# stulacy/bmm-mcmc

Measured on AMD Instinct MI355X. Metric: gibbs_sweeps_per_s, higher is better.
Workload: dtype f64; 1 GPU; c5: gibbs_collapsed K=20 N=10000000 P=100, 1 chain per GPU; sampler=collapsed, K=20, N=10000000, P=100, batch=2500000, chains=1, chains_per_gpu=1, burn_sweeps=30, x_layout=bit planes, ceil(P/32) words per observation, packed once at hand-over

## Files before the change

bmm-mcmc_amd/csrc/bmm_spec.h:

```cpp
#pragma once
#include <stdint.h>

#include "bmm_exp256.h"

#if defined(__HIPCC__)
#include <hip/hip_runtime.h>
#define BMM_HD __host__ __device__ __forceinline__
#else
#define BMM_HD inline
#endif

namespace bmm {

constexpr int kGroupW = 5;
constexpr int kGroupWAlt = 4;
constexpr int kGroupWm = 3;
constexpr int kGroupMm = 1 << kGroupWm;
constexpr int kOwnSub = 6;

enum : uint32_t {
    kStreamZ = 0,
    kStreamStickA = 1,
    kStreamStickB = 2,
    kStreamThetaA = 3,
// ... 326 lines not shown
    return n;
}

constexpr float kPkEpsUnit = 3.2f * 0x1p-24f;
constexpr float kPkLnCats = 4.1588831f;
BMM_HD float pk_band(float m, int G, float unit) {
    return unit * (80.0f + (float)(G + 2) * (__builtin_fabsf(m) + kPkLnCats + 1.0f));
}
template <int KT, class Exp2 = Exp2Fast>
BMM_HD bool draw_pk(const float (&sc)[KT], float m, double u, int G, float unit, int& cnt, Exp2 ex2 = Exp2()) {
    static_assert(KT <= kTier1MaxCats, "the band is derived for at most kTier1MaxCats categories");
    float c[KT];
    float run = 0.0f;
#if defined(__HIP_DEVICE_COMPILE__)
#pragma unroll
#endif
    for (int k = 0; k < KT; ++k) {
        run = run + ex2((sc[k] - m) * 0x1.715476p+0f);
        c[k] = run;
    }
    const float t = (float)u * run;
    float nearest = __builtin_inff();
    int n = 0;
#if defined(__HIP_DEVICE_COMPILE__)
#pragma unroll
#endif
    for (int k = 0; k < KT; ++k) {
        const float diff = t - c[k];
        n += diff >= 0.0f ? 1 : 0;
        nearest = __builtin_fminf(nearest, __builtin_fabsf(diff));
    }
    cnt = n;
    return nearest > pk_band(m, G, unit) * run && m > -__builtin_inff() && m < __builtin_inff();
}

BMM_HD double rnorm_(Stream& st) {
    for (;;) {
        const U4 r = st.next();
        const double v1 = 2.0 * u01(r.x, r.y) - 1.0, v2 = 2.0 * u01(r.z, r.w) - 1.0;
        const double s = v1 * v1 + v2 * v2;
        if (s < 1.0 && s > 0.0) return v1 * sqrt_(div_(-2.0 * log_(s), s));
    }
}

BMM_HD double rgamma_(double shape, Stream& st) {
    if (!(shape > 0.0)) return 0.0;
    double boost = 1.0;
    if (shape < 1.0) {
        const U4 r = st.next();
        boost = exp_(div_(log_(u01_open0(r.x, r.y)), shape));
        shape = shape + 1.0;
    }
    const double d = shape - 0.33333333333333331483;
    const double c = div_(1.0, sqrt_(9.0 * d));
    for (;;) {
        const double x = rnorm_(st);
        double v = 1.0 + c * x;
        if (v <= 0.0) continue;
        v = v * v * v;
        const U4 r = st.next();
        const double u = u01_open0(r.x, r.y);
        const double x2 = x * x;
        if (log_(u) < 0.5 * x2 + d - d * v + d * log_(v)) return d * v * boost;
    }
}

// ... 296 lines not shown
```

bmm-mcmc_amd/csrc/chain.hip:

```cpp
#include <hip/hip_runtime.h>
#include <hip/hip_ext.h>
#include <rccl/rccl.h>

#include <dlfcn.h>
#include <emmintrin.h>
#include <sched.h>
#include <sys/mman.h>

#include <algorithm>
#include <cmath>
#include <cstdarg>
#include <cstdio>
#include <cstdint>
#include <cstdlib>
#include <cstring>
#include <atomic>
#include <chrono>
#include <condition_variable>
#include <exception>
#include <functional>
#include <limits>
#include <memory>
#include <mutex>
#include <new>
// ... 428 lines not shown
    resample_fn fn = nullptr, fn_emit = nullptr;
    int grid_max_emit = 0;

    const int32_t* dX = nullptr;
    int32_t* dX_owned = nullptr;
    uint32_t* dXb = nullptr;
    struct Planes { uint32_t* d = nullptr; size_t bytes = 0; std::atomic<int> refs{1}; };
    Planes* planes = nullptr;
    bool xb_borrowed = false;
    bool bits = false;
    int num_cus = 0;
    char *arena = nullptr, *run_arena = nullptr;
    size_t arena_bytes = 0, run_arena_bytes = 0;
    int32_t* dZ[2] = {nullptr, nullptr};
    int32_t *dNk = nullptr, *dS = nullptr, *dDNk = nullptr, *dDS = nullptr;
    double *dAlpha = nullptr, *dTab = nullptr, *dPi = nullptr, *dTheta = nullptr;
    bool have_data = false, have_init = false, started = false;
    int sweep = 0;

    int burnin = 0, S = 0;
    int32_t* dTrace = nullptr;
    double *dThetaTrace = nullptr, *dAlphaTrace = nullptr, *dPiTrace = nullptr;
    char* dOutBlk[2] = {nullptr, nullptr};
    size_t out_blk_bytes = 0;

    int32_t* dNkTrace = nullptr;
    int nk_trace_base = 0;
    unsigned long long* dDiag = nullptr;
    int* dViable = nullptr;
    int* dSelfDone = nullptr;
    int32_t *dDNkAlt = nullptr, *dDSAlt = nullptr;
    unsigned long long* dPkStat = nullptr;
    int pk_defer_every = 0;
    int* dDbgFlag = nullptr;
    int64_t predM = 0;
    uint32_t* dXnb = nullptr;
    double *dPredTab = nullptr, *dPredMax = nullptr, *dPredSum = nullptr, *dRespAcc = nullptr;
    bool pred_resp = false;
    int pred_folded = 0;
    score_fn pfn = nullptr;
    int pred_grid_max = 0;
    size_t pred_lds = 0;
    SweepTrace pred_rec;
    int64_t pred_cells = 0;
    uint32_t* dPnMb = nullptr;
    int64_t *dPnRow = nullptr, *dPnOff = nullptr;
    int32_t* dPnCol = nullptr;
    double *dCellMax = nullptr, *dCellSum = nullptr, *dSplitTab = nullptr, *dPnScratch = nullptr;
    int64_t pn_scratch_stride = 0;
    na_score_fn pn_fn = nullptr;
    int pn_grid_max = 0;
    size_t pn_lds = 0;
    bool loo_on = false;
    double *dLooTab = nullptr, *dLooAcc = nullptr, *dLooOut = nullptr;
    bool loo_generic = false;
    double* dLooScratch = nullptr;
    int64_t loo_scratch_stride = 0;
    int loo_folded = 0;
    score_fn lfn = nullptr;
    int loo_minus = 0, loo_grid_max = 0;
    size_t loo_lds = 0;
    SweepTrace loo_rec;
    int sm_moves = 0, sm_scans = 0, sm_sets = 0;
    uint8_t *dSmSide = nullptr, *dSmSideLaunch = nullptr;
    double* dSmLq = nullptr;
    int32_t* dSmStat = nullptr;
// ... 203 lines not shown
    int flag = 0;
    hipError_t e = hipGetLastError();
    if (e == hipSuccess) e = hipMemcpyAsync(&flag, dflag, sizeof(int), hipMemcpyDeviceToHost, c->stream);
    if (e == hipSuccess) e = hipStreamSynchronize(c->stream);
    if (e != hipSuccess) return set_err(BMM_E_HIP, "validating X failed: %s", hipGetErrorString(e));
    if (flag) return set_err(BMM_E_ARG, "data must be binary: X holds a value other than 0 and 1");
    return BMM_OK;
}

constexpr int64_t kLargeN = (int64_t)1 << 16;
int64_t default_batch(int sampler, int64_t N) {
    if (sampler == BMM_SAMPLER_SB || sampler == BMM_SAMPLER_FULL) return N;
    const int64_t div = N >= kLargeN ? 4 : (sampler == BMM_SAMPLER_DP ? 16 : 8);
    const int64_t b = N / div;
    return b < 1 ? 1 : b;
}

TableLayout layout_of(const bmm_chain* c) { return layout_of(c->p, !explicit_params(c->p.mode)); }

int dbg_env_int(const char* name, int unset) { const char* v = dbg_env(name); return v ? (atoi(v) > 0 ? atoi(v) : 0) : unset; }
struct DebugSwitches {
    bool generic = dbg_env("BMM_DEBUG_GENERIC");
    bool int32_layout = dbg_env("BMM_X_LAYOUT_INT32");
    int cus = dbg_env_int("BMM_DEBUG_CUS", 0);
    int threads = dbg_env_int("BMM_DEBUG_THREADS", -1);
    bool split = dbg_env("BMM_DEBUG_SPLIT");
    bool nosplit = dbg_env("BMM_DEBUG_NOSPLIT");
    bool small = dbg_env("BMM_DEBUG_SMALL");
    bool noself = dbg_env("BMM_DEBUG_NOSELF");
    bool nopk = dbg_env("BMM_DEBUG_NOPK");
    bool pk = dbg_env("BMM_DEBUG_PK");
    bool nopipe = dbg_env("BMM_DEBUG_PK_NOPIPE");
    int pk_defer_every = dbg_env_int("BMM_DEBUG_PK_DEFER_EVERY", 0);
};

struct ChainShape {
    ChainParams p{};
    int64_t batch = 1;
    bool generic = false;
    int minus_in_lds = 1;
    size_t lds_bytes_base = 0;
};
ChainParams geometry(int sampler, int P, int K, int kt, int W) {
    ChainParams q{};
    q.mode = sampler; q.P = P; q.K = K; q.KT = kt; q.W = W;
    q.G = (P + W - 1) / W; q.Gm = (P + kGroupWm - 1) / kGroupWm;
    q.Kc = sampler == BMM_SAMPLER_DP ? K + 1 : K;
    return q;
}
size_t image_bytes(const ChainParams& q, bool own_tables) {
    const TableLayout l = layout_of(q, own_tables && !explicit_params(q.mode));
    return (size_t)(own_tables ? l.doubles() : l.head()) * sizeof(double) + ((size_t)q.K * q.P + q.K + 4) * sizeof(int32_t);
}

size_t pk_image_bytes(const ChainParams& q) {
    const TableLayout l = layout_of(q, true);
    return (size_t)(2 * pk_tq_doubles(l) + l.tm() - l.nk()) * sizeof(double) + ((size_t)q.K * q.P + q.K + 4 + kPkQueue) * sizeof(int32_t);
}

int group_width_rule(int sampler, int K, int P) {
    const int kt = pick_kt(sampler == BMM_SAMPLER_DP ? K + 1 : K);
    if (kt < 0 || P > kMaxP) return kGroupWAlt;
    return image_bytes(geometry(sampler, P, K, kt, kGroupW), true) <= kLdsMax ? kGroupW : kGroupWAlt;
}

int64_t generic_threads(int Kc) {
// ... 120 lines not shown
    int rc = chain_stream_create(c, true);
    if (rc) { c->stream = old; c->stream_kind = old_kind; return rc; }
    chain_stream_release(c->device, old, old_kind);
    return BMM_OK;
}

struct Carver {
    char* base;
    size_t used = 0;
    template <class T> T* take(size_t n) {
        const size_t off = (used + 255) & ~(size_t)255;
        used = off + n * sizeof(T);
        return base ? reinterpret_cast<T*>(base + off) : nullptr;
    }
};

int chain_alloc(bmm_chain* c) {
    const ChainParams& p = c->p;
    HIP_TRY(hipSetDevice(c->device));
    {
        int rcs = chain_stream_create(c, false);
        if (rcs) return rcs;
    }
    const size_t nz = (size_t)p.N;
    const size_t ns = (size_t)p.K * p.P, nn = (size_t)p.K;
    const size_t ntab = (size_t)layout_of(c).doubles() + (explicit_params(p.mode) ? 0 : 2 * (size_t)pk_tq_doubles(layout_of(c)));
    auto carve = [&](Carver& a) {
        c->dNk = a.take<int32_t>(nn);
        c->dDNk = a.take<int32_t>(nn * kDeltaReps);
        c->dS = a.take<int32_t>(ns);
        c->dDS = a.take<int32_t>(ns * kDeltaReps);
        c->dTab = a.take<double>(ntab);
#ifdef BMM_DIAG
        c->dDiag = a.take<unsigned long long>(18);
#endif
        c->dSelfDone = a.take<int>(1);
        c->dViable = a.take<int>(1);
        c->dDNkAlt = a.take<int32_t>(nn * kDeltaReps);
        c->dDSAlt = a.take<int32_t>(ns * kDeltaReps);
#ifdef BMM_DEBUG_HOOKS
        c->dDbgFlag = a.take<int>(1);
        c->dPkStat = a.take<unsigned long long>(3);
#endif
        const size_t zeroed = a.used;
        c->dAlpha = a.take<double>(1);
        c->dPi = a.take<double>(nn);
        c->dTheta = a.take<double>(ns);
        c->dZ[0] = a.take<int32_t>(nz);
        c->dZ[1] = a.take<int32_t>(nz);
        return zeroed;
    };
    Carver measure{nullptr};
    carve(measure);
    c->arena = static_cast<char*>(dev_pool().get(c->device, measure.used, &c->arena_bytes));
    if (!c->arena) return set_err(BMM_E_HIP, "allocating the chain's state failed: %s", hipGetErrorString(hipGetLastError()));
    Carver real{c->arena};
    const size_t zeroed = carve(real);
    if (c->generic) HIP_TRY(hipMalloc(&c->dScratch, (size_t)c->scratch_stride * p.Kc * sizeof(double)));
    HIP_TRY(hipMemsetAsync(c->arena, 0, zeroed, c->stream));
    HIP_TRY(hipMemsetAsync(c->dZ[0], 0xff, nz * sizeof(int32_t), c->stream));
    HIP_TRY(hipMemcpyAsync(c->dAlpha, &c->alpha0, sizeof(double), hipMemcpyHostToDevice, c->stream));
    HIP_TRY(hipStreamSynchronize(c->stream));
    return BMM_OK;
}

int dbg_labels_ok(bmm_chain* c) {
#ifdef BMM_DEBUG_HOOKS
    int flag = 0;
    HIP_TRY(hipMemcpy(&flag, c->dDbgFlag, sizeof(int), hipMemcpyDeviceToHost));
    if (flag) return set_err(BMM_E_STATE, "a resample kernel produced or read a label outside [0, K): kernel bug (debug-hooks build check)");
#else
    (void)c;
#endif
    return BMM_OK;
}

int launch_resample(bmm_chain* c, const int32_t* z_in, int32_t* z_out, int64_t lo, int64_t hi,
                    uint32_t sweep) {
    ResampleArgs a{};
    a.X = c->dX; a.Xb = c->dXb; a.z_in = z_in; a.z_out = z_out; a.tab = c->dTab; a.dNk = c->dDNk; a.dS = c->dDS;
    a.lo = lo; a.hi = hi; a.sweep = sweep; a.minus_in_lds = c->minus_in_lds; a.diag = c->dDiag;
    a.dbg_flag = c->dDbgFlag; a.dbg_inject = (dbg_env("BMM_DEBUG_BADLABEL") ? 1 : 0) | (dbg_env("BMM_DEBUG_STRAGGLER") ? 2 : 0) |
                                             (dbg_env("BMM_DEBUG_DRAW_FALLBACK") ? 4 : 0) | (dbg_env("BMM_DEBUG_DRAW_NOEPS") ? 8 : 0) |
                                             (dbg_env("BMM_DEBUG_PK_GENKEY") ? 16 : 0);
    a.Nk = c->dNk; a.S = c->dS; a.alpha_ptr = c->dAlpha; a.self_done = c->dSelfDone;
#ifdef BMM_DEBUG_HOOKS
    a.pk_stat = c->dPkStat;
    a.pk_defer_every = c->pk_defer_every;
#endif
    const bool emit = c->probs_dst != nullptr;
    const bool use_generic = c->generic || (emit && !c->fn_emit);
    const bool self_launch = c->form.self && !emit && !use_generic;
    if (self_launch) { a.dNk_prev = c->dDNk; a.dS_prev = c->dDS; a.dNk = c->dDNkAlt; a.dS = c->dDSAlt; }
    const KernelForm& form = emit ? c->form_emit : c->form;
    const int gmax = emit ? c->grid_max_emit : c->grid_max;
    const int64_t ntiles = use_generic ? 1 : (hi - lo + tile_of(form) - 1) / tile_of(form);
    int grid = (int)(ntiles < gmax ? ntiles : gmax);
    if (use_generic) {
        const int64_t nt256 = (hi - lo + 255) / 256;
        const int64_t maxb = c->scratch_stride / 256;
        grid = (int)(nt256 < maxb ? nt256 : maxb);
    }
    if (emit) { a.wts = c->dWts; a.wtot = c->dWtot; }
    if (form.pk && !use_generic) {
        a.Xb += lo;
        if (a.z_in) a.z_in += lo;
        a.z_out += lo;
    }
    hipEvent_t e0 = nullptr, e1 = nullptr;
    if (c->prof > 0 && sweep % (uint32_t)c->prof == 0) {
        if (c->ev_used + 2 > c->ev.size()) {
            hipEvent_t a0, a1;
            HIP_TRY(hipEventCreate(&a0));
            HIP_TRY(hipEventCreate(&a1));
            c->ev.push_back(a0); c->ev.push_back(a1);
        }
        e0 = c->ev[c->ev_used]; e1 = c->ev[c->ev_used + 1];
        c->ev_used += 2;
    }
    if (use_generic) {
        if (e0) hipExtLaunchKernelGGL(k_resample_generic, dim3(grid), dim3(256), 0, c->stream, e0, e1, 0, c->p, a,
// ... 923 lines not shown
        return set_err(BMM_E_ARG, "Error: sampler currently not implemented for non-symmetric priors on beta and gamma");
    if (sampler == BMM_SAMPLER_DP && K < 2) return set_err(BMM_E_ARG, "maxK must be >= 2");
    if (alpha < 0.0) return set_err(BMM_E_ARG, "alpha must be >= 0 (0 = sample it)");
    int ndev = 0;
    if (hipGetDeviceCount(&ndev) != hipSuccess || ndev < 1)
        return set_err(BMM_E_NODEVICE, "no HIP device visible; this path has no CPU fallback");
    const int slot = device;
    if (const int fake = fake_devices()) {
        if (device < 0 || device >= fake) return set_err(BMM_E_ARG, "device %d out of range (have %d)", device, fake);
        device = device % ndev;
    }
    if (device < 0 || device >= ndev) return set_err(BMM_E_ARG, "device %d out of range (have %d)", device, ndev);

    bmm_chain* c = new (std::nothrow) bmm_chain();
    if (!c) return set_err(BMM_E_ARG, "out of host memory");
    const DebugSwitches dbg;
    const ChainShape shape = chain_shape(sampler, N, P, K, batch, dbg);
    ChainParams& p = c->p;
    p = shape.p;
    p.beta = beta; p.gamma = gamma; p.a = a; p.b = b; p.seed = seed;
    p.sample_alpha = alpha == 0.0;
    c->alpha0 = p.sample_alpha ? 1.0 : alpha;
    c->device = device;
    c->slot = slot;
    c->batch = shape.batch;
    if (p.Kc > kMaxCatsAny) {
        delete c;
        return set_err(BMM_E_UNSUPPORTED, "%d categories exceed the %d this build supports", p.Kc, kMaxCatsAny);
    }
    const int cus = device_cus(device);
    if (cus <= 0) { delete c; return set_err(BMM_E_HIP, "hipGetDeviceProperties failed"); }
    c->bits = !dbg.int32_layout;
    c->pk_defer_every = dbg.pk_defer_every;
    c->generic = shape.generic;
    c->minus_in_lds = shape.minus_in_lds;
    c->lds_bytes_base = c->lds_bytes = shape.lds_bytes_base;
    if (c->generic) {
        c->form = KernelForm{p.KT, 256, tier_of(c), c->bits, 1, false, p.W, false};
        c->scratch_stride = generic_threads(p.Kc);
        c->grid_max = (int)(c->scratch_stride / 256);
    } else {
        c->num_cus = dbg.cus >= 1 ? dbg.cus : cus;
        rc = pick_kernel(c);
        if (rc) { delete c; return rc; }
    }
    rc = chain_alloc(c);
    if (rc) { bmm_chain_destroy(c); return rc; }
    *out = c;
    return BMM_OK;
}

void bmm_chain_destroy(bmm_chain* c) {
    if (!c) return;
    (void)hipSetDevice(c->device);
    if (c->stream) (void)hipStreamSynchronize(c->stream);
#ifdef BMM_DIAG
    if (c->dDiag) {
        unsigned long long d[18] = {};
        const bool ok = hipMemcpy(d, c->dDiag, sizeof d, hipMemcpyDeviceToHost) == hipSuccess;
        if (ok && d[5] && d[0]) {
            const double tot = (double)(d[0] + d[1] + d[2] + d[3] + d[4]);
            fprintf(stderr, "[bmm diag] waves=%llu cycles/wave: score %.0f (%.1f%%) pack %.0f (%.1f%%) draw %.0f (%.1f%%) movers %.0f (%.1f%%) prologue %.0f (%.1f%%) movers/wave-launch %.2f\n",
                    d[5], d[0] / (double)d[5], 100 * d[0] / tot, d[1] / (double)d[5], 100 * d[1] / tot, d[2] / (double)d[5],
                    100 * d[2] / tot, d[3] / (double)d[5], 100 * d[3] / tot, d[4] / (double)d[5], 100 * d[4] / tot, d[6] / (double)d[5]);
        }
        if (ok && d[5])
            fprintf(stderr, "[bmm diag launch] ticks per wave and launch: table staging %.0f, tile loop %.0f, waiting for the workgroup %.0f, flush %.0f\n",
                    d[8] / (double)d[5], d[9] / (double)d[5], d[10] / (double)d[5], d[11] / (double)d[5]);
        if (ok && d[7])
            fprintf(stderr, "[bmm diag launch pk] workgroup-launches %llu, ticks from entry to flushed %.0f\n", d[7], d[14] / (double)d[7]);
        if (ok && d[7] && d[17])
            fprintf(stderr, "[bmm diag trip pk] trips of wave 0: %llu, ticks per trip: scoring %.0f, outside it %.0f\n", d[17],
                    d[16] / (double)d[17], ((double)d[9] - (double)d[16]) / (double)d[17]);
        if (ok && d[5] && d[12])
            fprintf(stderr, "[bmm diag draw] draws of a wave (64 observations) %llu, of them by the binary64 definition %llu (%.4f%%)\n",
                    d[12], d[13], 100.0 * (double)d[13] / (double)d[12]);
    }
#endif
    for (hipEvent_t e : c->ev) (void)hipEventDestroy(e);
    if (c->planes && c->planes->refs.fetch_sub(1) == 1) {
        dev_pool().put(c->device, c->planes->d, c->planes->bytes);
        delete c->planes;
    }
    dev_pool().put(c->device, c->arena, c->arena_bytes);
    dev_pool().put(c->device, c->run_arena, c->run_arena_bytes);
    sum_release(c);
    void* bufs[] = {c->dX_owned, c->dScratch, c->dProbs, c->dWts, c->dWtot, c->dXnb, c->dPredTab, c->dPredMax, c->dPredSum, c->dRespAcc,
                    c->dLooTab, c->dLooAcc, c->dLooOut, c->dLooScratch, c->dSmSide, c->dSmSideLaunch, c->dSmLq, c->dSmStat, c->dSmCell,
                    c->dSmCounters, c->dFsBlock, c->dEaBlock, c->dEaSide, c->dAsBlock, c->dLjBlock, c->dLjZ, c->dPcFeat, c->dPcXt, c->dPcBlock, c->dNaBlock, c->dCsBlock, c->dCatBlock,
                    c->dPnMb, c->dPnRow, c->dPnOff, c->dPnCol, c->dCellMax, c->dCellSum, c->dSplitTab, c->dPnScratch};
    for (void* b : bufs)
        if (b) (void)hipFree(b);
    chain_stream_release(c->device, c->stream, c->stream_kind);
    delete c;
}

static int pack_rows(bmm_chain* c, const int32_t* dX, int64_t rows, int64_t ldx, int64_t i0) {
    const int64_t nb = (rows + 255) / 256;
    hipLaunchKernelGGL(k_pack_bits, dim3((unsigned)(nb < 16384 ? nb : 16384)), dim3(256), 0, c->stream, dX, rows,
                       ldx, c->p.P, c->dXb + i0, c->p.N);
    HIP_TRY(hipGetLastError());
    return BMM_OK;
}

int bmm_chain_set_x_layout(bmm_chain* c, int layout) {
    if (!c) return set_err(BMM_E_ARG, "null chain");
// ... 4466 lines not shown
extern "C" int bmm_dbg_host_labels(const void* src, int narrow, int32_t* dst, int64_t n, int jobs) {
    return guarded([&]() -> int {
        HostCrew crew;
        for (int j = 0; j < jobs; ++j) {
            if (narrow) crew.run(n, 256, 64, [=](int64_t lo, int64_t hi) { widen_labels(static_cast<const uint8_t*>(src) + lo, dst + lo, hi - lo); });
            else crew.run(n, 256, 64, [=](int64_t lo, int64_t hi) { copy_labels(static_cast<const int32_t*>(src) + lo, dst + lo, hi - lo); });
        }
        return BMM_OK;
    });
}
static void kernel_key(const KernelForm& f, const KernelForm& twin, bool generic, int grid_max_emit, int* key) {
    const int k[10] = {f.kt, f.nt, f.lanes, f.minus, f.bits ? 1 : 0, f.gw, f.self ? 1 : 0, generic ? 0 : twin.nt, generic ? 1 : 0, grid_max_emit};
    std::memcpy(key, k, sizeof k);
}
extern "C" int bmm_dbg_kernel_packed(const bmm_chain* c) { return c && !c->generic && c->form.pk ? 1 : 0; }
extern "C" int bmm_dbg_kernel_pk_pipelined(const bmm_chain* c) { return c && !c->generic && c->form.pk && c->form.pipe ? 1 : 0; }
extern "C" int bmm_dbg_pk_counts(bmm_chain* c, unsigned long long* draws, unsigned long long* deferred) {
    if (!c || !draws || !deferred) return set_err(BMM_E_ARG, "null argument");
    return guarded([&]() -> int {
        unsigned long long v[2] = {0, 0};
        HIP_TRY(hipSetDevice(c->device));
        HIP_TRY(hipStreamSynchronize(c->stream));
        HIP_TRY(hipMemcpy(v, c->dPkStat, sizeof v, hipMemcpyDeviceToHost));
        *draws = v[0]; *deferred = v[1];
        return BMM_OK;
    });
}
extern "C" int bmm_dbg_pk_unselected(bmm_chain* c, unsigned long long* n) {
    if (!c || !n) return set_err(BMM_E_ARG, "null argument");
    return guarded([&]() -> int {
        HIP_TRY(hipSetDevice(c->device));
        HIP_TRY(hipStreamSynchronize(c->stream));
        HIP_TRY(hipMemcpy(n, c->dPkStat + 2, sizeof *n, hipMemcpyDeviceToHost));
        return BMM_OK;
    });
}
extern "C" int bmm_dbg_kernel_key(const bmm_chain* c, int* key) {
    if (!c || !key) return set_err(BMM_E_ARG, "null argument");
    kernel_key(c->form, c->form_emit, c->generic, c->fn_emit ? c->grid_max_emit : 0, key);
    return BMM_OK;
}
extern "C" int bmm_dbg_kernel_plan(int sampler, int64_t N, int P, int K, int64_t batch, int num_cus, int shares_device,
                                   int int32_layout, int* key) {
    if (!key || sampler < 0 || sampler > 3 || N < 1 || P < 1 || K < 1 || num_cus < 1) return set_err(BMM_E_ARG, "bad argument");
    const DebugSwitches dbg;
    const ChainShape s = chain_shape(sampler, N, P, K, batch, dbg);
    const bool bits = !int32_layout && !dbg.int32_layout;
    const int minus = explicit_params(sampler) ? 0 : (s.minus_in_lds ? 1 : 2);
    if (s.generic) {
        kernel_key(KernelForm{s.p.KT, 256, minus, bits, 1, false, s.p.W, false}, KernelForm{}, true, 0, key);
        return BMM_OK;
    }
    const KernelPlan plan = plan_kernel(s.p, bits, minus, s.batch, dbg.cus >= 1 ? dbg.cus : num_cus, shares_device != 0,
                                        s.lds_bytes_base, dbg);
    const KernelForm& f = plan.form[plan.n - 1];
    kernel_key(f, bits ? emit_twin(f) : KernelForm{}, false, 0, key);
    return BMM_OK;
}
#endif

int st_run_check(const RunOptions& opts, int burnin, int K) {
    const bmm_relabel_out* const rel = opts.rel;
    if (!rel) return BMM_OK;
    if (!rel->permutations || !rel->z_original || !rel->theta_original) return set_err(BMM_E_ARG, "null buffer");
    if (burnin < 2 || rel->burnrelabel < 1)
        return set_err(BMM_E_ARG, "relabel on the device needs the batch step, which the reference runs only with "
// ... 1219 lines not shown
```

bmm-mcmc_amd/csrc/kernels.hip.h:

```cpp
#pragma once
#include <hip/hip_runtime.h>
#include <stdint.h>

#include <type_traits>

#include "bmm_spec.h"

namespace bmm {

typedef __attribute__((address_space(3))) double lds_f64;

constexpr int kMaxP = 128;
constexpr int lcm_(int a, int b) { int x = a; while (x % b) x += a; return x; }
constexpr int kChunkP = kMaxP / lcm_(lcm_(kGroupW, kGroupWAlt), kGroupWm) * lcm_(lcm_(kGroupW, kGroupWAlt), kGroupWm);
constexpr int kMaxCats = 64;
constexpr int kMaxCatsAny = 1024;

enum : int { MODE_COLLAPSED = 0, MODE_DP = 1, MODE_SB = 2, MODE_FULL = 3 };
__host__ __device__ inline bool explicit_params(int mode) { return mode == MODE_SB || mode == MODE_FULL; }

struct TableLayout {
    int G, KT, Gm, M;
    __host__ __device__ int tp() const { return 0; }
    __host__ __device__ int cp() const { return G * KT * M; }
// ... 487 lines not shown
        }
        if (threadIdx.x == 0) {
            if (p.sample_alpha) *alpha_ptr = al;
            if (alpha_trace) *alpha_trace = al;
        }
    }
}

struct ResampleArgs {
    const int32_t* X;
    const uint32_t* Xb;
    const int32_t* z_in;
    int32_t* z_out;
    const double* tab;
    int32_t* dNk;
    int32_t* dS;
    int64_t lo, hi;
    uint32_t sweep;
    int minus_in_lds;
    double* wts;
    double* wtot;
    unsigned long long* diag;
    int* dbg_flag;
    int dbg_inject;
    int32_t* Nk;
    int32_t* S;
    int32_t* dNk_prev;
    int32_t* dS_prev;
    const double* alpha_ptr;
    int* self_done;
    unsigned long long* pk_stat;
#ifdef BMM_DEBUG_HOOKS
    int pk_defer_every;
#endif
};

#ifdef BMM_DEBUG_HOOKS
__device__ __forceinline__ void dbg_check_labels(const ResampleArgs& a, bool valid, bool first, int K, int& zn, int& zo) {
    if ((a.dbg_inject & 1) && valid && first) zn = K + 3;
    if (valid && (zn < 0 || zn >= K || zo < -1 || zo >= K)) {
        atomicOr(a.dbg_flag, 1);
        zn = -1; zo = -1;
    }
}
#define BMM_DBG_LABELS(a, valid, first, K, zn, zo) dbg_check_labels(a, valid, first, K, zn, zo)
#define DBG_TIER1_FORCE(a, certain) if ((a).dbg_inject & 4) certain = false
#define DBG_TIER1_EPS(a, eps) if ((a).dbg_inject & 8) eps = 0.0f
#else
#define BMM_DBG_LABELS(a, valid, first, K, zn, zo)
#define DBG_TIER1_FORCE(a, certain)
#define DBG_TIER1_EPS(a, eps)
#endif

__device__ __forceinline__ double max_score(double m, double sc) {
    double r;
    asm("v_max_f64 %0, %1, %2" : "=v"(r) : "v"(m), "v"(sc));
    return r;
}

struct TilePos {
    const char* base;
    uint32_t voff;
    int64_t i, ic;
    bool valid;
};
__device__ __forceinline__ TilePos tile_pos(const ResampleArgs& a, int64_t tile, int NT, int tid, int lane) {
// ... 643 lines not shown
#pragma unroll 1
    for (int g0 = 0; g0 < G; g0 += GR) {
        double tv[GR];
#pragma unroll
        for (int v = 0; v < GR; ++v) {
            const int g = g0 + v < G ? g0 + v : G - 1;
            const double* const row = tp + ((size_t)g * KT * GM + (unsigned)__builtin_amdgcn_readlane(fld, g));
            tv[v] = row[koff];
        }
#pragma unroll
        for (int v = 0; v < GR; ++v)
            if (g0 + v < G) sc = sc + tv[v];
    }
    double own = 0.0;
#pragma unroll 1
    for (int g = 0; g < gmp; ++g) own = own + pk_bcast(oe, g);
    if (k == zo) sc = own;
    double m = neg_inf();
#pragma unroll
    for (int j = 0; j < KT; ++j) m = max_score(m, pk_bcast(sc, j));
    const double w = expw_tab(sc - m, ET);
    double run = 0.0, cdf = 0.0;
#pragma unroll
    for (int j = 0; j < KT; ++j) {
        run = run + pk_bcast(w, j);
        cdf = lane == j ? run : cdf;
    }
    const double t = u * run;
    int zn = (int)__popcll(__ballot(lane < KT && t >= cdf));
    if (!(m > neg_inf())) zn = zoc;
    return zn;
}

struct PkArgsView {
    const ChainParams* p;
    const ResampleArgs* a;
};
static_assert(alignof(ChainParams) == 8 && alignof(ResampleArgs) == 8 && sizeof(ChainParams) % 8 == 0,
              "k_resample_pk(ChainParams, ResampleArgs): the second argument lies right behind the first");
__device__ __forceinline__ PkArgsView pk_args_view() {
    const __attribute__((address_space(4))) char* ka =
        (const __attribute__((address_space(4))) char*)__builtin_amdgcn_kernarg_segment_ptr();
    asm volatile("" : "+s"(ka));
    PkArgsView v;
    v.p = (const ChainParams*)ka;
    v.a = (const ResampleArgs*)(ka + sizeof(ChainParams));
    return v;
}
struct PkLds {
    const int32_t* NkT;
    const lds_f64* ET;
    int32_t* hist;
};
__device__ __forceinline__ PkLds pk_lds(char* smem, const TableLayout& L) {
    double* const tail = reinterpret_cast<double*>(smem) + 2 * pk_tq_doubles(L);
    PkLds r;
    r.NkT = reinterpret_cast<const int32_t*>(tail);
    r.ET = (const lds_f64*)(tail + (L.et() - L.nk()));
    r.hist = reinterpret_cast<int32_t*>(tail + (L.tm() - L.nk()));
    return r;
}

struct PkPos {
    uint32_t s0;
    uint32_t loff;
    bool valid;
// ... 158 lines not shown
    asm volatile("" : "+s"(G));
#pragma unroll
    for (int j = 0; j < KP; ++j) acc[j] = pk_f2{0.0f, 0.0f};
    own32 = 0.0f;
    pk_step<KT, GW, 0>(Tq, orow0, b0, b1, b2, b3, acc, own32, head);
    pk_step_end<KT>(acc);
    bool whole = false;
    if constexpr (kRound0) whole = G >= KP;
    if (whole) {
        if constexpr (kRound0)
            pk_static_for<1, KP>([&](auto J) {
                pk_step<KT, GW, decltype(J)::value>(Tq, orow0, b0, b1, b2, b3, acc, own32, [] {});
                pk_step_end<KT>(acc);
            });
    } else if (G > 1) {
        pk_groups<KT, GW>(Tq, orow0, 1, G, W, b0, b1, b2, b3, acc, own32);
    }
    whole = false;
    if constexpr (kRound1) whole = G >= 2 * KP;
    if (whole) {
        if constexpr (kRound1)
            pk_static_for<0, KP>([&](auto J) {
                pk_step<KT, GW, KP + decltype(J)::value>(Tq, orow0, b0, b1, b2, b3, acc, own32, [] {});
                pk_step_end<KT>(acc);
            });
        if (G > 2 * KP) pk_groups<KT, GW>(Tq, orow0, 2 * KP, G, W, b0, b1, b2, b3, acc, own32);
    } else if (G > KP) {
        pk_groups<KT, GW>(Tq, orow0, KP, G, W, b0, b1, b2, b3, acc, own32);
    }
}

constexpr bool pk_pipelined(int kt, int nt, int ) { return nt == 1024 && kt <= 20; }

template <int KT, int GW>
__device__ __forceinline__ int pk_settle(const ResampleArgs& a, char* smem, const PkPos& pos, int lane, bool certain,
                                         int cnt, double u, int zo, uint32_t b0, uint32_t b1, uint32_t b2, uint32_t b3,
                                         int dp_K, int K, unsigned& ndeferred, unsigned& nunselected) {
    constexpr int GM = 1 << GW;
    const int zoc = zo < 0 ? 0 : zo;
    DBG_TIER1_FORCE(a, certain);
    bool defer = pos.valid && !certain;
#ifdef BMM_DEBUG_HOOKS
    const bool selected = a.pk_defer_every > 0 && pos.valid &&
                          (a.lo + (int64_t)pos.s0 + lane) % a.pk_defer_every == 0;
    nunselected += (unsigned)__popcll(__ballot(defer && !selected));
    defer = defer || selected;
#endif
    int zn = cnt;
    unsigned long long o = __ballot(defer);
#ifdef BMM_DEBUG_HOOKS
    ndeferred += (unsigned)__popcll(o);
#endif
    if (__builtin_expect(o != 0, 0)) {
        const PkArgsView v = pk_args_view();
        const TableLayout Lc{v.p->G, KT, v.p->Gm, GM};
        const PkLds lc = pk_lds(smem, Lc);
        int ln = lane;
        asm volatile("" : "+v"(ln));
        do {
            const int src = __ffsll((long long)o) - 1;
            o &= o - 1;
            const uint32_t w0 = __builtin_amdgcn_readlane(b0, src), w1 = __builtin_amdgcn_readlane(b1, src);
            const uint32_t w2 = __builtin_amdgcn_readlane(b2, src), w3 = __builtin_amdgcn_readlane(b3, src);
            const int e = pk_exact_count<KT, GW>(*v.p, *v.a, Lc, w0, w1, w2, w3, __builtin_amdgcn_readlane(zo, src),
                                                        pk_bcast(u, src), lc.ET, ln);
            if (ln == src) zn = e;
        } while (o);
    }
    if (__builtin_expect(__ballot(zn == dp_K) != 0, 0)) {
        const PkArgsView v = pk_args_view();
        const int Kc = v.p->K;
        const TableLayout Lc{v.p->G, KT, v.p->Gm, GM};
        const int32_t* const Nkc = pk_lds(smem, Lc).NkT;
        int Kused = 0, new_label = -1;
        for (int k = 0; k < Kc; ++k) {
            if (Nkc[k] > 0) ++Kused;
            else if (new_label < 0) new_label = k;
        }
        if (zn == Kc) zn = pk_dp_label(Nkc, Kc, Kused, new_label, zo, zoc);
    }
    const bool keep = pos.valid;
#ifdef BMM_DEBUG_HOOKS
    BMM_DBG_LABELS(a, keep, pos.s0 + (uint32_t)lane == 0u, K, zn, zo);
#endif
    const bool moves = keep && zn >= 0 && zn != zo;
    if (__builtin_expect(__ballot(moves) != 0, 0)) {
        const PkArgsView v = pk_args_view();
        const int Kc = v.p->K, Pc = v.p->P;
        const TableLayout Lc{v.p->G, KT, v.p->Gm, GM};
        int ln = lane;
        asm volatile("" : "+v"(ln));
        count_movers(moves, zo, zn, b0, b1, b2, b3, pk_lds(smem, Lc).hist, Kc, Pc, ln);
    }
    return zn;
}

template <int KT, int NT, int GW, bool PIPE>
__global__ __launch_bounds__(NT) void k_resample_pk(ChainParams p, ResampleArgs a) {
    static_assert(KT % 2 == 0 && KT <= 32, "pairs of categories, one lane per category in pk_exact_count");
    constexpr int GM = 1 << GW;
// ... 25 lines not shown
    uint32_t b0 = 0, b1 = 0, b2 = 0, b3 = 0;
    if (has_tile) pk_load_words(a.Xb, p.N, W, pos, b0, b1, b2, b3);
    {
        auto stage = [&](const double* from, double* to, int n2) {
            const double2* src = reinterpret_cast<const double2*>(from);
            double2* dst = reinterpret_cast<double2*>(to);
            for (int i0 = tid; i0 < n2; i0 += NT * 8) {
                double2 t[8];
#pragma unroll
                for (int u = 0; u < 8; ++u) {
                    const int i = i0 + u * NT;
                    t[u] = src[i < n2 ? i : n2 - 1];
                }
#pragma unroll
                for (int u = 0; u < 8; ++u) {
                    const int i = i0 + u * NT;
                    if (i < n2) dst[i] = t[u];
                }
            }
        };
        stage(a.tab + L.doubles(), lds, nq_d);
        stage(a.tab + L.nk(), tail, tail_d / 2);
    }
    for (int i = tid; i < K * P + K; i += NT) hist[i] = 0;
    if (tid == 0) *next_chunk = NW;
    __syncthreads();
    DIAG(const unsigned long long d_staged = diag_stamp();)
    DIAG(unsigned long long d_score = 0, d_trips = 0;)

    float unit = kPkEpsUnit;
#ifdef BMM_DEBUG_HOOKS
    if (a.dbg_inject & 8) unit = 0.0f;
#endif
    unsigned ndeferred = 0, nunselected = 0;

    if (has_tile) {
        const uint32_t* const Xb = a.Xb;
        const int32_t* const z_in = a.z_in;
        int32_t* const z_out = a.z_out;
        const int64_t N = p.N;
        const uint64_t seed = p.seed, i0 = (uint64_t)(p.obs0 + a.lo);
        const uint32_t sweep = a.sweep;
        int key_general = (int)(uint32_t)(((uint64_t)(p.obs0 + a.hi) - 1u) >> 32);
#ifdef BMM_DEBUG_HOOKS
        if (a.dbg_inject & 16) key_general = 1;
#endif
        key_general = __builtin_amdgcn_readfirstlane(key_general);
        const int dp_K = p.mode == MODE_DP ? K : -1;
        const int has_zin = (int)((uint32_t)((uintptr_t)z_in >> 32) | (uint32_t)(uintptr_t)z_in);
        int zo = -1;
        if (z_in) zo = *pk_at(z_in + pos.s0, pos.loff);
        asm volatile("" : "+v"(zo));
        if constexpr (!PIPE) {
        int zn_prev = 0;
        uint32_t st_s0 = 0, st_loff = 0;
        bool st_on = false;
        for (;;) {
            const int zoc = zo < 0 ? 0 : zo;
            if (st_on) *pk_at(z_out + st_s0, st_loff) = zn_prev;
            int nc = 0;
            if (lane == 0) nc = atomicAdd(next_chunk, 1);
            nc = __builtin_amdgcn_readfirstlane(nc);
            const bool has_next = nc < wg_cn;
            const PkPos npos = pk_pos(n, has_next ? wg_c0 + nc : 0, lane);
            uint32_t n0 = 0, n1 = 0, n2 = 0, n3 = 0;
            int zo_next = -1;
            int Wl = W, zl = has_zin;
// ... 23 lines not shown
                    const volatile lds_f32* orow = orow0 + ((size_t)g * KT * GM + nib);
#pragma unroll
                    for (int c0 = 0; c0 < KP; c0 += CH) {
                        pk_f2 tv[CH];
                        float ov = 0.0f;
#pragma unroll
                        for (int j = 0; j < CH; ++j) tv[j] = row[(c0 + j) * GM];
                        if (c0 == 0) ov = *orow;
#pragma unroll
                        for (int j = 0; j < CH; ++j) acc[c0 + j] = acc[c0 + j] + tv[j];
                        if (c0 == 0) own32 = own32 + ov;
                        if (CH < KP) __builtin_amdgcn_sched_barrier(0);
                    }
                }
            }
            __builtin_amdgcn_s_setprio(0);
            DIAG(d_score += diag_stamp() - d_s0; ++d_trips;)
            pk_f2 s2[KP];
            float m = -__builtin_inff();
#pragma unroll
            for (int j = 0; j < KP; ++j) {
                float x = acc[j].x, y = acc[j].y;
                if (2 * j == zo) x = own32;
                if (2 * j + 1 == zo) y = own32;
                s2[j] = pk_f2{x, y};
                m = __builtin_fmaxf(m, x);
                m = __builtin_fmaxf(m, y);
            }
            int kg = key_general;
            asm volatile("" : "+s"(kg));
            const double u = pk_uniform(seed, i0, pos.s0, pos.loff, sweep, kg == 0);
            int cnt = 0;
            const bool certain = pk_draw2<KT>(s2, m, u, G, unit, cnt);
            const int zn = pk_settle<KT, GW>(a, smem, pos, lane, certain, cnt, u, zo, b0, b1, b2, b3, dp_K, K, ndeferred,
                                             nunselected);
            const bool keep = pos.valid;
            zn_prev = zn;
            st_s0 = pos.s0; st_loff = pos.loff; st_on = keep;
            if (!has_next) break;
            b0 = n0; b1 = n1; b2 = n2; b3 = n3;
            zo = zo_next;
            pos = npos;
        }
        if (st_on) *pk_at(z_out + st_s0, st_loff) = zn_prev;
        } else {
        int zn_prev = 0;
        uint32_t st_s0 = 0, st_loff = 0;
        bool st_on = false;
        for (;;) {
            const int zoc = zo < 0 ? 0 : zo;
            if (st_on) *pk_at(z_out + st_s0, st_loff) = zn_prev;
            int nc = 0;
            if (lane == 0) nc = atomicAdd(next_chunk, 1);
            bool has_next = false;
            PkPos npos;
            npos.s0 = pos.s0; npos.loff = pos.loff; npos.valid = pos.valid;
            uint32_t n0 = 0, n1 = 0, n2 = 0, n3 = 0;
            int zo_next = -1;
            double u = 0.0;
            int Wl = W, zl = has_zin, kg = key_general;
            asm volatile("" : "+s"(Wl), "+s"(zl), "+s"(kg));
            pk_f2 acc[KP];
            float own32;
            const volatile lds_f32* const orow0 = Tm32 + zoc * GM;
            DIAG(const unsigned long long d_s0 = diag_stamp();)
            __builtin_amdgcn_s_setprio(BMM_LOOKUP_PRIO);
            pk_score<KT, GW>(Tq, orow0, G, W, b0, b1, b2, b3, acc, own32, [&] {
                __builtin_amdgcn_sched_barrier(0);
                nc = __builtin_amdgcn_readfirstlane(nc);
                has_next = nc < wg_cn;
                const PkPos t = pk_pos(n, has_next ? wg_c0 + nc : 0, lane);
                npos.s0 = t.s0; npos.loff = t.loff; npos.valid = t.valid;
                if (has_next) {
                    pk_load_words(Xb, N, Wl, npos, n0, n1, n2, n3);
                    if (zl) zo_next = *pk_at(z_in + npos.s0, npos.loff);
                }
                u = pk_uniform(seed, i0, pos.s0, pos.loff, sweep, kg == 0);
            });
            __builtin_amdgcn_s_setprio(0);
            DIAG(d_score += diag_stamp() - d_s0; ++d_trips;)
            pk_f2 s2[KP];
            float m = -__builtin_inff();
#pragma unroll
            for (int j = 0; j < KP; ++j) {
                float x = acc[j].x, y = acc[j].y;
                if (2 * j == zo) x = own32;
                if (2 * j + 1 == zo) y = own32;
                s2[j] = pk_f2{x, y};
                m = __builtin_fmaxf(m, x);
                m = __builtin_fmaxf(m, y);
            }
            int cnt = 0;
            const bool certain = pk_draw2<KT>(s2, m, u, G, unit, cnt);
            const int zn = pk_settle<KT, GW>(a, smem, pos, lane, certain, cnt, u, zo, b0, b1, b2, b3, dp_K, K, ndeferred,
                                             nunselected);
            zn_prev = zn;
            st_s0 = pos.s0; st_loff = pos.loff; st_on = pos.valid;
            if (!has_next) break;
            b0 = n0; b1 = n1; b2 = n2; b3 = n3;
            zo = zo_next;
            pos.s0 = npos.s0; pos.loff = npos.loff; pos.valid = npos.valid;
        }
        if (st_on) *pk_at(z_out + st_s0, st_loff) = zn_prev;
        }
    }

    DIAG(const unsigned long long d_loop = diag_stamp();)
    __syncthreads();
    DIAG(const unsigned long long d_sync = diag_stamp();)
    {
        const PkArgsView v = pk_args_view();
        const int Kc = v.p->K, Pc = v.p->P;
        const TableLayout Lc{v.p->G, KT, v.p->Gm, GM};
        const int rep = blockIdx.x % kDeltaReps;
        flush_hist(pk_lds(smem, Lc).hist, Kc, Pc, v.a->dS + (size_t)rep * Kc * Pc, v.a->dNk + rep * Kc, tid, NT);
    }
    DIAG(asm volatile("s_waitcnt vmcnt(0)" ::: "memory"); const unsigned long long d_flush = diag_stamp();)
    DIAG(if (a.diag && tid == 0) {
        atomicAdd(&a.diag[5], 1ull); atomicAdd(&a.diag[7], 1ull); atomicAdd(&a.diag[14], d_flush - d_entry);
        atomicAdd(&a.diag[8], d_staged - d_entry); atomicAdd(&a.diag[9], d_loop - d_staged);
        atomicAdd(&a.diag[10], d_sync - d_loop); atomicAdd(&a.diag[11], d_flush - d_sync);
        atomicAdd(&a.diag[16], d_score); atomicAdd(&a.diag[17], d_trips);
    })
#ifdef BMM_DEBUG_HOOKS
    if (a.pk_stat) {
        if (tid == 0) {
            int64_t first = a.lo + (int64_t)wg_c0 * 64, last = a.lo + ((int64_t)wg_c0 + (wg_cn > 0 ? wg_cn : 0)) * 64;
            last = last < a.hi ? last : a.hi;
            if (last > first) atomicAdd(&a.pk_stat[0], (unsigned long long)(last - first));
        }
        if (lane == 0 && ndeferred) atomicAdd(&a.pk_stat[1], (unsigned long long)ndeferred);
        if (lane == 0 && nunselected) atomicAdd(&a.pk_stat[2], (unsigned long long)nunselected);
    }
#endif
}

__device__ __forceinline__ unsigned field_from_x(const int32_t* X, const uint32_t* Xb, int64_t N, int P,
                                                  int64_t i, int g, int GW) {
    if (Xb) {
        const int o = g * GW, w = o >> 5, sh = o & 31, W = (P + 31) >> 5;
        uint32_t v = Xb[(int64_t)w * N + i] >> sh;
        if (sh + GW > 32 && w + 1 < W) v |= Xb[(int64_t)(w + 1) * N + i] << (32 - sh);
        return v & (unsigned)((1 << GW) - 1);
    }
    unsigned nib = 0;
    for (int j = 0; j < GW; ++j) {
        const int d = g * GW + j;
        if (d < P) nib |= ((unsigned)X[i + (int64_t)d * N] & 1u) << j;
    }
    return nib;
}

__global__ __launch_bounds__(256) void k_resample_generic(ChainParams p, ResampleArgs a, double* scr,
                                                          int64_t stride) {
    const bool has_minus = !explicit_params(p.mode);
    const TableLayout L = layout_of(p, has_minus);
    const int GM = L.M;
    const double* const Tp = a.tab + L.tp();
    const double* const Tm = a.tab + L.tm();
    const int32_t* const NkT = reinterpret_cast<const int32_t*>(a.tab + L.nk());
    const double* const ET = a.tab + L.et();
    const int P = p.P, G = p.G, K = p.K, Kc = p.Kc, KT = p.KT;
    const int64_t gid = (int64_t)blockIdx.x * blockDim.x + threadIdx.x;
    double* const my = scr + gid;

// ... 3199 lines not shown
```

Baseline: 3972 sweeps/s.

## Add a middle-tier f32-table/f64-sum draw before the exact fallback for deferred observations

```diff
diff --git a/bmm-mcmc_amd/csrc/bmm_spec.h b/bmm-mcmc_amd/csrc/bmm_spec.h
--- a/bmm-mcmc_amd/csrc/bmm_spec.h
+++ b/bmm-mcmc_amd/csrc/bmm_spec.h
@@ -382,6 +382,39 @@
     }
     cnt = n;
     return nearest > pk_band(m, G, unit) * run && m > -__builtin_inff() && m < __builtin_inff();
+}
+
+constexpr double kMidEpsUnit = 4.8 * 0x1p-24;
+constexpr double kMidC0 = 1.0;
+constexpr double kMidLnCats = 4.1588830833596715;
+BMM_HD double mid_band(double m, double unit) {
+    return unit * (kMidC0 + 2.0 * (__builtin_fabs(m) + kMidLnCats + 1.0));
+}
+template <int KT, int GMAX>
+BMM_HD bool draw_mid(const float (&e)[GMAX][KT], int G, double u, double unit, int& cnt) {
+    static_assert(KT <= kTier1MaxCats, "the band is derived for at most kTier1MaxCats categories");
+    double sc[KT], c[KT];
+    double m = neg_inf();
+    bool nan = false;
+    for (int k = 0; k < KT; ++k) {
+        double a = 0.0;
+        for (int g = 0; g < G; ++g) a = a + (double)e[g][k];
+        sc[k] = a;
+        nan = nan || a != a;
+        m = __builtin_fmax(m, a);
+    }
+    double run = 0.0;
+    for (int k = 0; k < KT; ++k) { run = run + expw_(sc[k] - m); c[k] = run; }
+    const double t = u * run;
+    const double band = mid_band(m, unit) * run;
+    bool clear = true;
+    int n = 0;
+    for (int k = 0; k < KT; ++k) {
+        n += t >= c[k] ? 1 : 0;
+        clear = clear && __builtin_fabs(t - c[k]) > band;
+    }
+    cnt = n;
+    return clear && !nan && m > neg_inf() && m < pos_inf();
 }
 
 BMM_HD double rnorm_(Stream& st) {
diff --git a/bmm-mcmc_amd/csrc/chain.hip b/bmm-mcmc_amd/csrc/chain.hip
--- a/bmm-mcmc_amd/csrc/chain.hip
+++ b/bmm-mcmc_amd/csrc/chain.hip
@@ -484,6 +484,7 @@
     int32_t *dDNkAlt = nullptr, *dDSAlt = nullptr;
     unsigned long long* dPkStat = nullptr;
     int pk_defer_every = 0;
+    int pk_mid_fail_every = 0;
     int* dDbgFlag = nullptr;
     int64_t predM = 0;
     uint32_t* dXnb = nullptr;
@@ -753,6 +754,7 @@
     bool pk = dbg_env("BMM_DEBUG_PK");
     bool nopipe = dbg_env("BMM_DEBUG_PK_NOPIPE");
     int pk_defer_every = dbg_env_int("BMM_DEBUG_PK_DEFER_EVERY", 0);
+    int pk_mid_fail_every = dbg_env_int("BMM_DEBUG_PK_MID_FAIL_EVERY", 0);
 };
 
 struct ChainShape {
@@ -939,7 +941,7 @@
         c->dDS = a.take<int32_t>(ns * kDeltaReps);
         c->dTab = a.take<double>(ntab);
 #ifdef BMM_DIAG
-        c->dDiag = a.take<unsigned long long>(18);
+        c->dDiag = a.take<unsigned long long>(22);
 #endif
         c->dSelfDone = a.take<int>(1);
         c->dViable = a.take<int>(1);
@@ -947,7 +949,7 @@
         c->dDSAlt = a.take<int32_t>(ns * kDeltaReps);
 #ifdef BMM_DEBUG_HOOKS
         c->dDbgFlag = a.take<int>(1);
-        c->dPkStat = a.take<unsigned long long>(3);
+        c->dPkStat = a.take<unsigned long long>(6);
 #endif
         const size_t zeroed = a.used;
         c->dAlpha = a.take<double>(1);
@@ -989,11 +991,12 @@
     a.lo = lo; a.hi = hi; a.sweep = sweep; a.minus_in_lds = c->minus_in_lds; a.diag = c->dDiag;
     a.dbg_flag = c->dDbgFlag; a.dbg_inject = (dbg_env("BMM_DEBUG_BADLABEL") ? 1 : 0) | (dbg_env("BMM_DEBUG_STRAGGLER") ? 2 : 0) |
                                              (dbg_env("BMM_DEBUG_DRAW_FALLBACK") ? 4 : 0) | (dbg_env("BMM_DEBUG_DRAW_NOEPS") ? 8 : 0) |
-                                             (dbg_env("BMM_DEBUG_PK_GENKEY") ? 16 : 0);
+                                             (dbg_env("BMM_DEBUG_PK_GENKEY") ? 16 : 0) | (dbg_env("BMM_DEBUG_PK_NOMID") ? 32 : 0);
     a.Nk = c->dNk; a.S = c->dS; a.alpha_ptr = c->dAlpha; a.self_done = c->dSelfDone;
 #ifdef BMM_DEBUG_HOOKS
     a.pk_stat = c->dPkStat;
     a.pk_defer_every = c->pk_defer_every;
+    a.pk_mid_fail_every = c->pk_mid_fail_every;
 #endif
     const bool emit = c->probs_dst != nullptr;
     const bool use_generic = c->generic || (emit && !c->fn_emit);
@@ -1983,6 +1986,7 @@
     if (cus <= 0) { delete c; return set_err(BMM_E_HIP, "hipGetDeviceProperties failed"); }
     c->bits = !dbg.int32_layout;
     c->pk_defer_every = dbg.pk_defer_every;
+    c->pk_mid_fail_every = dbg.pk_mid_fail_every;
     c->generic = shape.generic;
     c->minus_in_lds = shape.minus_in_lds;
     c->lds_bytes_base = c->lds_bytes = shape.lds_bytes_base;
@@ -2007,7 +2011,7 @@
     if (c->stream) (void)hipStreamSynchronize(c->stream);
 #ifdef BMM_DIAG
     if (c->dDiag) {
-        unsigned long long d[18] = {};
+        unsigned long long d[22] = {};
         const bool ok = hipMemcpy(d, c->dDiag, sizeof d, hipMemcpyDeviceToHost) == hipSuccess;
         if (ok && d[5] && d[0]) {
             const double tot = (double)(d[0] + d[1] + d[2] + d[3] + d[4]);
@@ -2023,6 +2027,19 @@
         if (ok && d[7] && d[17])
             fprintf(stderr, "[bmm diag trip pk] trips of wave 0: %llu, ticks per trip: scoring %.0f, outside it %.0f\n", d[17],
                     d[16] / (double)d[17], ((double)d[9] - (double)d[16]) / (double)d[17]);
+        if (ok && d[7] && (d[19] || d[21]))
+            fprintf(stderr, "[bmm diag settle pk] wave 0 per workgroup-launch: middle tier runs %.4f at %.0f ticks each, definition runs %.4f at %.0f ticks each, "
+                    "together %.0f ticks of the tile loop's %.0f (%.2f%%)\n",
+                    d[19] / (double)d[7], d[19] ? d[18] / (double)d[19] : 0.0, d[21] / (double)d[7], d[21] ? d[20] / (double)d[21] : 0.0,
+                    (double)(d[18] + d[20]) / (double)d[7], d[9] / (double)d[5], 100.0 * (double)(d[18] + d[20]) / (double)d[9]);
+#ifdef BMM_DEBUG_HOOKS
+        if (ok && d[7] && c->dPkStat) {
+            unsigned long long v[6] = {};
+            if (hipMemcpy(v, c->dPkStat, sizeof v, hipMemcpyDeviceToHost) == hipSuccess && v[0])
+                fprintf(stderr, "[bmm diag tiers pk] draws %llu deferred %llu (%.4f%%) middle tier tried %llu settled %llu definition runs %llu\n", v[0],
+                        v[1], 100.0 * (double)v[1] / (double)v[0], v[3], v[4], v[5]);
+        }
+#endif
         if (ok && d[5] && d[12])
             fprintf(stderr, "[bmm diag draw] draws of a wave (64 observations) %llu, of them by the binary64 definition %llu (%.4f%%)\n",
                     d[12], d[13], 100.0 * (double)d[13] / (double)d[12]);
@@ -6555,6 +6572,18 @@
         HIP_TRY(hipSetDevice(c->device));
         HIP_TRY(hipStreamSynchronize(c->stream));
         HIP_TRY(hipMemcpy(n, c->dPkStat + 2, sizeof *n, hipMemcpyDeviceToHost));
+        return BMM_OK;
+    });
+}
+extern "C" int bmm_dbg_pk_tier_counts(bmm_chain* c, unsigned long long* mid_tried, unsigned long long* mid_settled,
+                                      unsigned long long* exact_runs) {
+    if (!c || !mid_tried || !mid_settled || !exact_runs) return set_err(BMM_E_ARG, "null argument");
+    return guarded([&]() -> int {
+        unsigned long long v[3] = {0, 0, 0};
+        HIP_TRY(hipSetDevice(c->device));
+        HIP_TRY(hipStreamSynchronize(c->stream));
+        HIP_TRY(hipMemcpy(v, c->dPkStat + 3, sizeof v, hipMemcpyDeviceToHost));
+        *mid_tried = v[0]; *mid_settled = v[1]; *exact_runs = v[2];
         return BMM_OK;
     });
 }
diff --git a/bmm-mcmc_amd/csrc/kernels.hip.h b/bmm-mcmc_amd/csrc/kernels.hip.h
--- a/bmm-mcmc_amd/csrc/kernels.hip.h
+++ b/bmm-mcmc_amd/csrc/kernels.hip.h
@@ -543,6 +543,7 @@
     unsigned long long* pk_stat;
 #ifdef BMM_DEBUG_HOOKS
     int pk_defer_every;
+    int pk_mid_fail_every;
 #endif
 };
 
@@ -1252,6 +1253,94 @@
     return zn;
 }
 
+template <int CTRL, int ROWS>
+__device__ __forceinline__ double pk_dpp(double old, double x) {
+    const long long o = __double_as_longlong(old), b = __double_as_longlong(x);
+    const uint32_t lo = (uint32_t)__builtin_amdgcn_update_dpp((int)(uint32_t)o, (int)(uint32_t)b, CTRL, ROWS, 0xf, false);
+    const uint32_t hi = (uint32_t)__builtin_amdgcn_update_dpp((int)(uint32_t)(o >> 32), (int)(uint32_t)(b >> 32), CTRL, ROWS, 0xf, false);
+    return __longlong_as_double((long long)(((uint64_t)hi << 32) | lo));
+}
+
+template <int GW, int g>
+__device__ __forceinline__ unsigned pk_field_at(uint32_t w0, uint32_t w1, uint32_t w2, uint32_t w3) {
+    constexpr int bit = g * GW, wd = bit >> 5, sh = bit & 31;
+    static_assert(bit + GW <= kMaxP, "a group of the pattern");
+    const uint32_t lo = wd == 0 ? w0 : (wd == 1 ? w1 : (wd == 2 ? w2 : w3));
+    const uint32_t hi = wd == 0 ? w1 : (wd == 1 ? w2 : (wd == 2 ? w3 : 0u));
+    const uint32_t f = sh + GW <= 32 ? lo >> sh : (lo >> sh) | (hi << ((32 - sh) & 31));
+    return f & (unsigned)((1 << GW) - 1);
+}
+
+template <int KT, int GW>
+__device__ __forceinline__ int pk_mid_count(const TableLayout& L, int G, const char* smem, uint32_t w0, uint32_t w1,
+                                            uint32_t w2, uint32_t w3, int zo, double u, const lds_f64* ET, int lane,
+                                            bool& certain) {
+    constexpr int GM = 1 << GW;
+    constexpr int MR = KT <= 4 ? 6 : KT <= 8 ? 10 : 20;
+    static_assert(KT <= 32, "the walks cover two rows of 16 lanes");
+    static_assert((kMaxP + GW - 1) / GW <= 64, "lane g holds the field of group g");
+    const lds_f32* const img = (const lds_f32*)smem;
+    const int k = lane < KT ? lane : KT - 1;
+    const bool is_own = lane == zo;
+    const unsigned base = is_own ? 2u * (unsigned)pk_tq_doubles(L) + (unsigned)k * GM : (unsigned)(k >> 1) * (2 * GM) + (unsigned)(k & 1);
+    const unsigned fsh = is_own ? 0u : 1u;
+    double part[4] = {0.0, 0.0, 0.0, 0.0};
+    int g_from = 0;
+    if (G >= MR) {
+        static_assert(MR * GW <= kMaxP, "the first round's groups exist");
+        float tv[MR];
+        pk_static_for<0, MR>([&](auto J) {
+            constexpr int g = decltype(J)::value;
+            tv[g] = img[(unsigned)g * (KT * GM) + (base + (pk_field_at<GW, g>(w0, w1, w2, w3) << fsh))];
+        });
+        pk_static_for<0, MR>([&](auto J) {
+            constexpr int g = decltype(J)::value;
+            part[g & 3] = part[g & 3] + (double)tv[g];
+        });
+        g_from = MR;
+    }
+    int fld = 0;
+    if (g_from < G) {
+        const int gl = lane < G ? lane : G - 1;
+        fld = (int)pk_field(gl * GW, GM - 1, w0, w1, w2, w3);
+    }
+#pragma unroll 1
+    for (int g0 = g_from; g0 < G; g0 += MR) {
+        float tv[MR];
+#pragma unroll
+        for (int v = 0; v < MR; ++v) {
+            const int g = g0 + v < G ? g0 + v : G - 1;
+            tv[v] = img[(unsigned)g * (KT * GM) + base + ((unsigned)__builtin_amdgcn_readlane(fld, g) << fsh)];
+        }
+#pragma unroll
+        for (int v = 0; v < MR; ++v)
+            if (g0 + v < G) part[v & 3] = part[v & 3] + (double)tv[v];
+    }
+    double sc = (part[0] + part[1]) + (part[2] + part[3]);
+    if (lane >= KT) sc = neg_inf();
+    const bool nan = __ballot(sc != sc) != 0;
+    double m = sc;
+    m = __builtin_fmax(m, pk_dpp<0x111, 0xf>(m, m));
+    m = __builtin_fmax(m, pk_dpp<0x112, 0xf>(m, m));
+    m = __builtin_fmax(m, pk_dpp<0x114, 0xf>(m, m));
+    m = __builtin_fmax(m, pk_dpp<0x118, 0xf>(m, m));
+    m = __builtin_fmax(m, pk_dpp<0x142, 0xa>(m, m));
+    m = pk_bcast(m, 31);
+    double cdf = lane < KT ? expw_tab(sc - m, ET) : 0.0;
+    cdf = cdf + pk_dpp<0x111, 0xf>(0.0, cdf);
+    cdf = cdf + pk_dpp<0x112, 0xf>(0.0, cdf);
+    cdf = cdf + pk_dpp<0x114, 0xf>(0.0, cdf);
+    cdf = cdf + pk_dpp<0x118, 0xf>(0.0, cdf);
+    cdf = cdf + pk_dpp<0x142, 0xa>(0.0, cdf);
+    const double tot = pk_bcast(cdf, 31);
+    const double t = u * tot;
+    const double band = mid_band(m, kMidEpsUnit) * tot;
+    const int cnt = (int)__popcll(__ballot(lane < KT && t >= cdf));
+    const bool close = __ballot(lane < KT && !(__builtin_fabs(t - cdf) > band)) != 0;
+    certain = !close && !nan && m > neg_inf() && m < pos_inf();
+    return cnt;
+}
+
 struct PkArgsView {
     const ChainParams* p;
     const ResampleArgs* a;
@@ -1476,10 +1565,17 @@
 
 constexpr bool pk_pipelined(int kt, int nt, int ) { return nt == 1024 && kt <= 20; }
 
+struct PkTally {
+    unsigned deferred = 0, unselected = 0;
+    unsigned mid_tried = 0, mid_settled = 0, exact = 0;
+    DIAG(unsigned long long t_mid = 0, t_exact = 0;)
+    DIAG(unsigned n_mid = 0, n_exact = 0;)
+};
+
 template <int KT, int GW>
 __device__ __forceinline__ int pk_settle(const ResampleArgs& a, char* smem, const PkPos& pos, int lane, bool certain,
                                          int cnt, double u, int zo, uint32_t b0, uint32_t b1, uint32_t b2, uint32_t b3,
-                                         int dp_K, int K, unsigned& ndeferred, unsigned& nunselected) {
+                                         int dp_K, int K, PkTally& tally) {
     constexpr int GM = 1 << GW;
     const int zoc = zo < 0 ? 0 : zo;
     DBG_TIER1_FORCE(a, certain);
@@ -1487,13 +1583,13 @@
 #ifdef BMM_DEBUG_HOOKS
     const bool selected = a.pk_defer_every > 0 && pos.valid &&
                           (a.lo + (int64_t)pos.s0 + lane) % a.pk_defer_every == 0;
-    nunselected += (unsigned)__popcll(__ballot(defer && !selected));
+    tally.unselected += (unsigned)__popcll(__ballot(defer && !selected));
     defer = defer || selected;
 #endif
     int zn = cnt;
     unsigned long long o = __ballot(defer);
 #ifdef BMM_DEBUG_HOOKS
-    ndeferred += (unsigned)__popcll(o);
+    tally.deferred += (unsigned)__popcll(o);
 #endif
     if (__builtin_expect(o != 0, 0)) {
         const PkArgsView v = pk_args_view();
@@ -1501,15 +1597,41 @@
         const PkLds lc = pk_lds(smem, Lc);
         int ln = lane;
         asm volatile("" : "+v"(ln));
+        __builtin_amdgcn_s_setprio(3);
         do {
             const int src = __ffsll((long long)o) - 1;
             o &= o - 1;
             const uint32_t w0 = __builtin_amdgcn_readlane(b0, src), w1 = __builtin_amdgcn_readlane(b1, src);
             const uint32_t w2 = __builtin_amdgcn_readlane(b2, src), w3 = __builtin_amdgcn_readlane(b3, src);
-            const int e = pk_exact_count<KT, GW>(*v.p, *v.a, Lc, w0, w1, w2, w3, __builtin_amdgcn_readlane(zo, src),
-                                                        pk_bcast(u, src), lc.ET, ln);
+            const int zs = __builtin_amdgcn_readlane(zo, src);
+            const double us = pk_bcast(u, src);
+            bool settled = false;
+            int e = 0;
+            bool try_mid = true;
+#ifdef BMM_DEBUG_HOOKS
+            if (v.a->dbg_inject & 32) try_mid = false;
+#endif
+            if (try_mid) {
+                DIAG(const unsigned long long d_m0 = diag_stamp();)
+                e = pk_mid_count<KT, GW>(Lc, v.p->G, smem, w0, w1, w2, w3, zs, us, lc.ET, ln, settled);
+                DIAG(tally.t_mid += diag_stamp() - d_m0; ++tally.n_mid;)
+#ifdef BMM_DEBUG_HOOKS
+                if (v.a->pk_mid_fail_every > 0 && (v.a->lo + (int64_t)pos.s0 + src) % v.a->pk_mid_fail_every == 0) settled = false;
+                ++tally.mid_tried;
+                tally.mid_settled += settled ? 1u : 0u;
+#endif
+            }
+            if (!settled) {
+                DIAG(const unsigned long long d_e0 = diag_stamp();)
+                e = pk_exact_count<KT, GW>(*v.p, *v.a, Lc, w0, w1, w2, w3, zs, us, lc.ET, ln);
+                DIAG(tally.t_exact += diag_stamp() - d_e0; ++tally.n_exact;)
+#ifdef BMM_DEBUG_HOOKS
+                ++tally.exact;
+#endif
+            }
             if (ln == src) zn = e;
         } while (o);
+        __builtin_amdgcn_s_setprio(0);
     }
     if (__builtin_expect(__ballot(zn == dp_K) != 0, 0)) {
         const PkArgsView v = pk_args_view();
@@ -1601,7 +1723,7 @@
 #ifdef BMM_DEBUG_HOOKS
     if (a.dbg_inject & 8) unit = 0.0f;
 #endif
-    unsigned ndeferred = 0, nunselected = 0;
+    PkTally tally;
 
     if (has_tile) {
         const uint32_t* const Xb = a.Xb;
@@ -1691,8 +1813,7 @@
             const double u = pk_uniform(seed, i0, pos.s0, pos.loff, sweep, kg == 0);
             int cnt = 0;
             const bool certain = pk_draw2<KT>(s2, m, u, G, unit, cnt);
-            const int zn = pk_settle<KT, GW>(a, smem, pos, lane, certain, cnt, u, zo, b0, b1, b2, b3, dp_K, K, ndeferred,
-                                             nunselected);
+            const int zn = pk_settle<KT, GW>(a, smem, pos, lane, certain, cnt, u, zo, b0, b1, b2, b3, dp_K, K, tally);
             const bool keep = pos.valid;
             zn_prev = zn;
             st_s0 = pos.s0; st_loff = pos.loff; st_on = keep;
@@ -1751,8 +1872,7 @@
             }
             int cnt = 0;
             const bool certain = pk_draw2<KT>(s2, m, u, G, unit, cnt);
-            const int zn = pk_settle<KT, GW>(a, smem, pos, lane, certain, cnt, u, zo, b0, b1, b2, b3, dp_K, K, ndeferred,
-                                             nunselected);
+            const int zn = pk_settle<KT, GW>(a, smem, pos, lane, certain, cnt, u, zo, b0, b1, b2, b3, dp_K, K, tally);
             zn_prev = zn;
             st_s0 = pos.s0; st_loff = pos.loff; st_on = pos.valid;
             if (!has_next) break;
@@ -1780,6 +1900,8 @@
         atomicAdd(&a.diag[8], d_staged - d_entry); atomicAdd(&a.diag[9], d_loop - d_staged);
         atomicAdd(&a.diag[10], d_sync - d_loop); atomicAdd(&a.diag[11], d_flush - d_sync);
         atomicAdd(&a.diag[16], d_score); atomicAdd(&a.diag[17], d_trips);
+        if (tally.n_mid) { atomicAdd(&a.diag[18], tally.t_mid); atomicAdd(&a.diag[19], (unsigned long long)tally.n_mid); }
+        if (tally.n_exact) { atomicAdd(&a.diag[20], tally.t_exact); atomicAdd(&a.diag[21], (unsigned long long)tally.n_exact); }
     })
 #ifdef BMM_DEBUG_HOOKS
     if (a.pk_stat) {
@@ -1788,8 +1910,11 @@
             last = last < a.hi ? last : a.hi;
             if (last > first) atomicAdd(&a.pk_stat[0], (unsigned long long)(last - first));
         }
-        if (lane == 0 && ndeferred) atomicAdd(&a.pk_stat[1], (unsigned long long)ndeferred);
-        if (lane == 0 && nunselected) atomicAdd(&a.pk_stat[2], (unsigned long long)nunselected);
+        if (lane == 0 && tally.deferred) atomicAdd(&a.pk_stat[1], (unsigned long long)tally.deferred);
+        if (lane == 0 && tally.unselected) atomicAdd(&a.pk_stat[2], (unsigned long long)tally.unselected);
+        if (lane == 0 && tally.mid_tried) atomicAdd(&a.pk_stat[3], (unsigned long long)tally.mid_tried);
+        if (lane == 0 && tally.mid_settled) atomicAdd(&a.pk_stat[4], (unsigned long long)tally.mid_settled);
+        if (lane == 0 && tally.exact) atomicAdd(&a.pk_stat[5], (unsigned long long)tally.exact);
     }
 #endif
 }
```

Measured after the change: 4171 sweeps/s (median of 6 runs). 5.0% higher.
